# shubhamchandak94/Spring

Hardware: AMD Instinct MI355X
Metric: Mreads/s through reorder stage (higher is better)
Workload: dtype u64; 1 GPU; 100000000 x 150 bp single-end synthetic reads per GPU (uniform genome 600000000 bp, 25x coverage, 1.0% substitutions, 50% reverse-complemented), inputs resident in HBM as .dna records; reads_per_gpu=100000000, read_len=150, chains=65536, num_thr=8, parallelism=single GPU, unmatched=13958636, singletons=12720853, rounds=1984, chain_groups=2

## Files before the change

### include/spring_reorder.h

```cpp
#ifndef SPRING_REORDER_H_
#define SPRING_REORDER_H_

#include <stddef.h>
#include <stdint.h>

#ifdef __cplusplus
extern "C" {
#endif

#define SPRING_REORDER_E_ARG (-1)
#define SPRING_REORDER_E_IO (-2)
#define SPRING_REORDER_E_HIP (-3)
#define SPRING_REORDER_E_STATE (-4)

typedef struct spring_reorder_ctx spring_reorder_ctx;

typedef struct {
  int32_t device;
  uint32_t num_chains;
  int32_t num_thr;
  int32_t collect_stats;
  int32_t time_search;
  int32_t force_literal_update;
  int32_t rounds_per_sync;
// ... 22 lines not shown
  int32_t phases;
  int32_t known_absent;
  int32_t sort_prefix_bits;
  int32_t dict_build_mode;
  int32_t strand_filter;
} spring_reorder_opts;

typedef struct {
  uint64_t n_reads, n_matched, n_single, unmatched;
  uint64_t probes, keyok, cands, hits, iterations, rounds, lost;
  uint64_t numkeys[2], dict_numreads[2];
  double ms_unpack, ms_dict, ms_chains, ms_finalize, ms_total;
  double ms_search_kernel;
  uint64_t search_launches;
  uint64_t device_bytes;
  double ms_exchange, ms_resolve_mark;
  uint64_t chains;
  uint64_t deep_pool;
  uint64_t long_searches;
  uint64_t table_minz;
  uint64_t table_marked_lines;
  uint64_t long_splits;
  uint64_t alternatives;
  uint64_t phases;
  double ms_search_busy;
  uint64_t sort_prefix_bits;
  uint64_t sort_repaired_runs;
  uint64_t sort_full_sorts;
  uint64_t sort_long_runs;
  uint64_t sort_list_overflows;
  uint64_t dict_build_path;
  uint64_t strand_filter;
  uint64_t strand_filter_dropped;
} spring_reorder_stats;

void spring_reorder_default_opts(spring_reorder_opts *o);
const char *spring_reorder_last_error(void);
void spring_reorder_trim_pool(void);

int spring_reorder_run(const char *temp_dir, uint32_t max_readlen, int32_t num_thr, int32_t paired_end,
                       uint32_t num_reads_clean_0, uint32_t num_reads_clean_1,
                       const spring_reorder_opts *opts );

int spring_reorder_create(spring_reorder_ctx **ctx, const spring_reorder_opts *opts);
void spring_reorder_destroy(spring_reorder_ctx *ctx);

int spring_reorder_load_dna(spring_reorder_ctx *ctx, const uint8_t *dna, size_t nbytes, uint32_t n,
                            uint32_t max_readlen);

int spring_reorder_load_dna_device(spring_reorder_ctx *ctx, const void *d_dna, size_t nbytes, uint32_t n,
                                   uint32_t max_readlen, int32_t fixed_len);

int spring_reorder_build_dict(spring_reorder_ctx *ctx);

int spring_reorder_run_chains(spring_reorder_ctx *ctx);
int spring_reorder_auto_chains(spring_reorder_ctx *ctx, uint32_t *chains, int32_t *deep);

typedef struct {
  uint32_t num_reads[2], num_reads_clean[2], num_reads_N[2];
  uint32_t max_readlen;
  uint32_t pad;
  double ms_device;
} spring_fastq_info;
int spring_reorder_load_fastq(spring_reorder_ctx *ctx, const uint8_t *fastq_1, size_t nbytes_1, const uint8_t *fastq_2,
                              size_t nbytes_2 , spring_fastq_info *info);
int spring_reorder_fastq_N(spring_reorder_ctx *ctx, int32_t which, uint8_t *n_dna, size_t cap, size_t *nbytes,
// ... 4 lines not shown
int spring_reorder_mg_slice(spring_reorder_ctx *ctx, void **d_prop, size_t *slice_off, size_t *slice_bytes,
                            size_t *total_bytes);
int spring_reorder_mg_slices(spring_reorder_ctx *ctx, void **d_prop, size_t slice_off[2], size_t slice_bytes[2],
                             size_t *total_bytes, uint32_t *count);
int spring_reorder_mg_apply(spring_reorder_ctx *ctx, int32_t check_alive, uint32_t *alive);
int spring_reorder_mg_end(spring_reorder_ctx *ctx);
int spring_reorder_debug_check_seed_state(spring_reorder_ctx *ctx, int32_t group, uint64_t *violations);
int spring_reorder_mg_exchange_virtual(spring_reorder_ctx **ctxs, uint32_t world);

#define SPRING_RCCL_ID_BYTES 128
typedef struct spring_mg_comm spring_mg_comm;
typedef int (*spring_mg_allgather_fn)(void *host_buf, size_t slice_off, size_t slice_bytes, size_t total_bytes,
                                      void *user);
int spring_mg_rccl_unique_id(void *id128);
int spring_mg_comm_create_rccl(spring_mg_comm **comm, int32_t device, const void *id128, uint32_t rank, uint32_t world);
int spring_mg_comm_create_host(spring_mg_comm **comm, spring_mg_allgather_fn fn, void *user, uint32_t rank,
                               uint32_t world);
void spring_mg_comm_destroy(spring_mg_comm *comm);
int spring_reorder_mg_run(spring_reorder_ctx *ctx, spring_mg_comm *comm, uint32_t total_chains);

int spring_reorder_finalize(spring_reorder_ctx *ctx);

int spring_reorder_get_stats(spring_reorder_ctx *ctx, spring_reorder_stats *st);

int spring_reorder_download(spring_reorder_ctx *ctx, uint32_t *order, char *rc, char *flag, int64_t *pos,
                            uint16_t *rlen, uint32_t *order_s, uint64_t *tid_off, uint64_t *tid_off_s);
int spring_reorder_tid_split(spring_reorder_ctx *ctx, uint64_t *mid, uint64_t *mid_s);

int spring_reorder_emit_dna(spring_reorder_ctx *ctx, int32_t tid, uint8_t *dst, size_t cap, size_t *nbytes);

int spring_reorder_dict_lookup(spring_reorder_ctx *ctx, int32_t which, const uint64_t *keys, uint32_t nkeys,
                               uint32_t *bin_size, uint32_t *bin_ids, size_t ids_cap);

int spring_reorder_download_reads(spring_reorder_ctx *ctx, uint64_t *limbs , uint16_t *len);

int spring_order_invert_se(const uint32_t *order, uint32_t n, uint32_t *order_array, double *kernel_ms);
int spring_order_invert_pe(const uint32_t *order, uint32_t n, uint32_t *order_array, double *kernel_ms);
int spring_order_correct(uint32_t *order, uint64_t m, const uint32_t *order_N, uint32_t nN, uint32_t n_clean,
                         double *kernel_ms);
int spring_order_pe_encode(const uint32_t *order, uint32_t n, uint32_t *new_order, double *kernel_ms);

int spring_fastq_reorder(const uint8_t *fastq, size_t nbytes, const uint32_t *order, uint32_t n, uint8_t *out,
                         size_t out_cap, size_t *out_bytes, double *kernel_ms);

#define SPRING_SYNTH_REPEATS 0x80000000u
#define SPRING_SYNTH_PAIRED 0x40000000u
#define SPRING_SYNTH_GENOMIC 0x20000000u
size_t spring_synth_dna_bytes(uint32_t n, uint32_t L);
int spring_synth_dna_host(uint8_t *dst, uint32_t n, uint32_t L, uint64_t G, uint64_t seed, uint32_t err_ppm);
int spring_synth_genome_host(uint8_t *dst, uint64_t G, uint64_t seed, uint32_t flags);
int spring_synth_dna_device(void *d_dst, uint32_t n, uint32_t L, uint64_t G, uint64_t seed, uint32_t err_ppm);
int spring_reorder_load_synth(spring_reorder_ctx *ctx, uint32_t n, uint32_t L, uint64_t G, uint64_t seed,
                              uint32_t err_ppm);
int spring_reorder_download_dna(spring_reorder_ctx *ctx, uint8_t *dst, size_t cap);

#ifdef __cplusplus
}
#endif
#endif
```

### spring_amd/_lib.py

```python
import ctypes as C
import os

HERE = os.path.dirname(os.path.abspath(__file__))
LIB_PATH = os.environ.get("SPRING_AMD_LIB") or os.path.join(HERE, "lib", "libspring_reorder_hip.so")

EXPORTS = [
    "spring_reorder_default_opts", "spring_reorder_last_error", "spring_reorder_trim_pool", "spring_reorder_run", "spring_reorder_create",
    "spring_reorder_destroy", "spring_reorder_load_dna", "spring_reorder_load_dna_device",
    "spring_reorder_build_dict", "spring_reorder_run_chains", "spring_reorder_auto_chains", "spring_reorder_finalize",
    "spring_reorder_mg_begin", "spring_reorder_mg_search", "spring_reorder_mg_slice", "spring_reorder_mg_slices",
    "spring_reorder_mg_apply",
    "spring_reorder_mg_end", "spring_reorder_mg_exchange_virtual", "spring_reorder_debug_check_seed_state",
    "spring_mg_rccl_unique_id", "spring_mg_comm_create_rccl", "spring_mg_comm_create_host", "spring_mg_comm_destroy",
    "spring_reorder_mg_run",
    "spring_reorder_get_stats", "spring_reorder_download", "spring_reorder_tid_split", "spring_reorder_emit_dna",
    "spring_reorder_dict_lookup", "spring_reorder_download_reads", "spring_synth_dna_bytes",
    "spring_reorder_load_fastq", "spring_reorder_fastq_N",
    "spring_order_invert_se", "spring_order_invert_pe", "spring_order_correct", "spring_order_pe_encode",
    "spring_fastq_reorder",
    "spring_synth_dna_host", "spring_synth_genome_host", "spring_synth_dna_device", "spring_reorder_load_synth", "spring_reorder_download_dna",
    "spring_encoder_create", "spring_encoder_destroy", "spring_encoder_set_split_tables", "spring_encoder_encode_reorder", "spring_encoder_download",
    "spring_encoder_download_seq_packed", "spring_encoder_get_info", "spring_reorder_encode_run", "spring_encoder_encode_host", "spring_encoder_run",
]

STREAMS_EXPORTS = [
    "spring_streams_create", "spring_streams_destroy", "spring_streams_from_encoder", "spring_streams_from_host",
    "spring_streams_download", "spring_streams_get_info", "spring_streams_run",
]
STREAMS_NUM = 9

DECODE_EXPORTS = [
    "spring_decode_create", "spring_decode_destroy", "spring_decode_seq_from_encoder", "spring_decode_seq_from_host",
    "spring_decode_seq_from_files", "spring_decode_from_streams", "spring_decode_from_host", "spring_decode_from_files",
    "spring_decode_download", "spring_decode_get_info",
]

QUALID_EXPORTS = [
    "spring_qualid_create", "spring_qualid_destroy", "spring_qualid_order_from_host", "spring_qualid_order_from_encoder",
    "spring_qualid_from_fastq", "spring_qualid_from_lines", "spring_qualid_download", "spring_qualid_get_info",
    "spring_quality_table", "spring_id_pattern",
]

FASTQ_OUT_EXPORTS = [
    "spring_fastq_out_create", "spring_fastq_out_destroy", "spring_fastq_out_assemble", "spring_fastq_out_download",
    "spring_fastq_out_write", "spring_fastq_out_get_info",
]

GZIP_EXPORTS = [
    "spring_gzip_create", "spring_gzip_destroy", "spring_gzip_set_chunk_bytes", "spring_gzip_set_token_bytes",
# ... 132 lines not shown
        for k, _ in self._fields_:
            v = getattr(self, k)
            d[k] = list(v) if hasattr(v, "__len__") else v
        return d


class DecodeInfo(C.Structure):
    _fields_ = ([(k, C.c_uint64) for k in ("seq_len", "first_block", "num_blocks", "num_units")]
                + [("bases", C.c_uint64 * 2)]
                + [(k, C.c_uint64) for k in ("n_aligned", "n_unaligned", "pos_escapes")]
                + [("ms_device", C.c_double), ("ms_file", C.c_double)])

    def asdict(self):
        d = {}
        for k, _ in self._fields_:
            v = getattr(self, k)
            d[k] = list(v) if hasattr(v, "__len__") else v
        return d


class Stats(C.Structure):
    _fields_ = ([(k, C.c_uint64) for k in ("n_reads", "n_matched", "n_single", "unmatched", "probes", "keyok",
                                          "cands", "hits", "iterations", "rounds", "lost")]
                + [("numkeys", C.c_uint64 * 2), ("dict_numreads", C.c_uint64 * 2)]
                + [(k, C.c_double) for k in ("ms_unpack", "ms_dict", "ms_chains", "ms_finalize", "ms_total",
                                             "ms_search_kernel")]
                + [("search_launches", C.c_uint64), ("device_bytes", C.c_uint64),
                   ("ms_exchange", C.c_double), ("ms_resolve_mark", C.c_double), ("chains", C.c_uint64),
                   ("deep_pool", C.c_uint64), ("long_searches", C.c_uint64),
                   ("table_minz", C.c_uint64), ("table_marked_lines", C.c_uint64), ("long_splits", C.c_uint64), ("alternatives", C.c_uint64), ("phases", C.c_uint64),
                   ("ms_search_busy", C.c_double),
                   ("sort_prefix_bits", C.c_uint64), ("sort_repaired_runs", C.c_uint64), ("sort_full_sorts", C.c_uint64),
                   ("sort_long_runs", C.c_uint64), ("sort_list_overflows", C.c_uint64), ("dict_build_path", C.c_uint64),
                   ("strand_filter", C.c_uint64), ("strand_filter_dropped", C.c_uint64)])

    def asdict(self):
        d = {}
        for k, _ in self._fields_:
            v = getattr(self, k)
            d[k] = list(v) if hasattr(v, "__len__") else v
        return d


MG_ALLGATHER_FN = C.CFUNCTYPE(C.c_int, C.c_void_p, C.c_size_t, C.c_size_t, C.c_size_t, C.c_void_p)

_lib = None


def lib():
    global _lib
    if _lib is not None:
        return _lib
    if not os.path.exists(LIB_PATH):
        raise RuntimeError(
            "spring_amd: %s is missing. Build it with `python -m spring_amd.build` "
            "(or __graft_entry__.build()); there is no CPU fallback." % LIB_PATH)
    L = C.CDLL(LIB_PATH)
    vp, u8p = C.c_void_p, C.c_void_p
    L.spring_reorder_default_opts.argtypes = [C.POINTER(Opts)]
    L.spring_reorder_last_error.restype = C.c_char_p
    L.spring_reorder_trim_pool.restype = None
    L.spring_reorder_run.argtypes = [C.c_char_p, C.c_uint32, C.c_int32, C.c_int32, C.c_uint32, C.c_uint32,
                                     C.POINTER(Opts)]
    L.spring_reorder_create.argtypes = [C.POINTER(vp), C.POINTER(Opts)]
    L.spring_reorder_destroy.argtypes = [vp]
    L.spring_reorder_destroy.restype = None
    L.spring_reorder_load_dna.argtypes = [vp, u8p, C.c_size_t, C.c_uint32, C.c_uint32]
    L.spring_reorder_load_dna_device.argtypes = [vp, vp, C.c_size_t, C.c_uint32, C.c_uint32, C.c_int32]
    L.spring_reorder_build_dict.argtypes = [vp]
    L.spring_reorder_run_chains.argtypes = [vp]
    L.spring_reorder_auto_chains.argtypes = [vp, C.POINTER(C.c_uint32), C.POINTER(C.c_int32)]
    L.spring_reorder_finalize.argtypes = [vp]
    L.spring_reorder_mg_begin.argtypes = [vp, C.c_uint32, C.c_uint32, C.c_uint32, vp]
    L.spring_reorder_mg_search.argtypes = [vp]
    L.spring_reorder_mg_slice.argtypes = [vp, C.POINTER(vp), C.POINTER(C.c_size_t), C.POINTER(C.c_size_t), C.POINTER(C.c_size_t)]
    L.spring_reorder_mg_slices.argtypes = [vp, C.POINTER(vp), C.POINTER(C.c_size_t), C.POINTER(C.c_size_t), C.POINTER(C.c_size_t),
                                           C.POINTER(C.c_uint32)]
    L.spring_reorder_debug_check_seed_state.argtypes = [vp, C.c_int32, C.POINTER(C.c_uint64)]
    L.spring_reorder_mg_apply.argtypes = [vp, C.c_int32, C.POINTER(C.c_uint32)]
    L.spring_reorder_mg_end.argtypes = [vp]
    L.spring_reorder_mg_exchange_virtual.argtypes = [C.POINTER(vp), C.c_uint32]
    L.spring_mg_rccl_unique_id.argtypes = [vp]
    L.spring_mg_comm_create_rccl.argtypes = [C.POINTER(vp), C.c_int32, vp, C.c_uint32, C.c_uint32]
    L.spring_mg_comm_create_host.argtypes = [C.POINTER(vp), MG_ALLGATHER_FN, vp, C.c_uint32, C.c_uint32]
    L.spring_mg_comm_destroy.argtypes = [vp]
    L.spring_mg_comm_destroy.restype = None
    L.spring_reorder_mg_run.argtypes = [vp, vp, C.c_uint32]
    L.spring_reorder_get_stats.argtypes = [vp, C.POINTER(Stats)]
    L.spring_reorder_download.argtypes = [vp] + [vp] * 8
    L.spring_reorder_tid_split.argtypes = [vp, vp, vp]
    L.spring_reorder_emit_dna.argtypes = [vp, C.c_int32, u8p, C.c_size_t, C.POINTER(C.c_size_t)]
    L.spring_reorder_dict_lookup.argtypes = [vp, C.c_int32, vp, C.c_uint32, vp, vp, C.c_size_t]
    L.spring_reorder_download_reads.argtypes = [vp, vp, vp]
    L.spring_reorder_load_fastq.argtypes = [vp, vp, C.c_size_t, vp, C.c_size_t, C.POINTER(FastqInfo)]
    L.spring_reorder_fastq_N.argtypes = [vp, C.c_int32, vp, C.c_size_t, C.POINTER(C.c_size_t), vp, C.POINTER(C.c_uint32)]
    L.spring_order_invert_se.argtypes = [vp, C.c_uint32, vp, C.POINTER(C.c_double)]
    L.spring_order_invert_pe.argtypes = [vp, C.c_uint32, vp, C.POINTER(C.c_double)]
    L.spring_fastq_reorder.argtypes = [u8p, C.c_size_t, vp, C.c_uint32, u8p, C.c_size_t, C.POINTER(C.c_size_t),
                                       C.POINTER(C.c_double)]
    L.spring_order_pe_encode.argtypes = [vp, C.c_uint32, vp, C.POINTER(C.c_double)]
    L.spring_order_correct.argtypes = [vp, C.c_uint64, vp, C.c_uint32, C.c_uint32, C.POINTER(C.c_double)]
    L.spring_synth_dna_bytes.restype = C.c_size_t
    L.spring_synth_dna_bytes.argtypes = [C.c_uint32, C.c_uint32]
    L.spring_synth_dna_host.argtypes = [u8p, C.c_uint32, C.c_uint32, C.c_uint64, C.c_uint64, C.c_uint32]
    L.spring_synth_genome_host.argtypes = [u8p, C.c_uint64, C.c_uint64, C.c_uint32]
    L.spring_synth_dna_device.argtypes = [vp, C.c_uint32, C.c_uint32, C.c_uint64, C.c_uint64, C.c_uint32]
    L.spring_reorder_load_synth.argtypes = [vp, C.c_uint32, C.c_uint32, C.c_uint64, C.c_uint64, C.c_uint32]
    L.spring_reorder_download_dna.argtypes = [vp, u8p, C.c_size_t]
    L.spring_encoder_create.argtypes = [C.c_int32, C.POINTER(vp)]
    L.spring_encoder_destroy.argtypes = [vp]
    L.spring_encoder_destroy.restype = None
    L.spring_encoder_encode_reorder.argtypes = [vp, vp, u8p, C.c_uint64, vp, C.c_uint32, C.POINTER(EncoderInfo)]
    L.spring_encoder_download.argtypes = [vp] + [vp] * 9
    L.spring_encoder_download_seq_packed.argtypes = [vp, vp, vp]
    L.spring_encoder_encode_host.argtypes = [vp, C.c_uint32, C.c_int32, vp, u8p, C.c_uint64, vp, vp, vp, vp, vp, u8p,
                                             C.c_uint64, vp, C.c_uint32, u8p, C.c_uint64, vp, C.c_uint32,
                                             C.POINTER(EncoderInfo)]
    L.spring_encoder_run.argtypes = [C.c_char_p, C.c_uint32, C.c_int32, C.c_uint32, C.c_uint32, C.c_int32,
                                     C.POINTER(EncoderInfo)]
    L.spring_encoder_get_info.argtypes = [vp, C.POINTER(EncoderInfo)]
    L.spring_reorder_encode_run.argtypes = [C.c_char_p, C.c_uint32, C.c_int32, C.c_int32, C.c_uint32, C.c_uint32,
                                            C.c_uint32, C.POINTER(Opts), C.POINTER(EncoderInfo)]
    L.spring_streams_create.argtypes = [C.c_int32, C.POINTER(vp)]
    L.spring_streams_destroy.argtypes = [vp]
    L.spring_streams_destroy.restype = None
# ... 105 lines not shown
```

### spring_amd/csrc/dict_build.h

```cpp
#ifndef SPRING_DICT_BUILD_H_
#define SPRING_DICT_BUILD_H_

#include "reorder_device.h"

namespace sr {

bool launch_unpack_keys(hipStream_t st, const uint8_t *dna, uint32_t n, int L, int W, int S, uint32_t rec_fixed,
                        uint64_t *reads, uint16_t *lens, uint32_t *bad_len, int dstart0, int dend0, int dstart1, int dend1,
                        uint64_t *keys0, uint32_t *vals0, uint64_t *keys1, uint32_t *vals1);

constexpr int TAB_WRITE_LG = 10;
inline int tab_write_lg(int bshift) { return 64 - bshift < TAB_WRITE_LG ? 64 - bshift : TAB_WRITE_LG; }
inline uint32_t tab_write_blocks(int bshift) { return (uint32_t)(1ull << (64 - bshift - tab_write_lg(bshift))); }
void launch_tab_partition(hipStream_t st, const uint64_t *h0, uint32_t nk0, const uint64_t *h1, uint32_t nk1, int bshift,
                          uint32_t *part);
constexpr uint32_t TAB_OVF_SLOTS = 8;
void launch_tab_write(hipStream_t st, const uint64_t *h0, uint32_t nk0, const uint64_t *h1, uint32_t nk1,
                      const uint32_t *part, DictBuild d0, DictBuild d1, uint4 *fpt, int bshift, uint32_t *ovf,
                      uint32_t *ovf_blk, uint32_t *ovf_cnt);
void launch_tab_overflow_blocks(hipStream_t st, const uint64_t *h0, uint32_t nk0, const uint64_t *h1, DictBuild d0,
                                DictBuild d1, uint32_t *fpt, int bshift, const uint32_t *ovf_blk, const uint32_t *ovf_cnt);
void launch_tab_overflow_pairs(hipStream_t st, const uint64_t *h0, uint32_t nk0, const uint64_t *h1, DictBuild d0,
                               DictBuild d1, uint32_t *fpt, int bshift, const uint32_t *ovf, uint32_t novf);

constexpr uint32_t PRES_DROP_CTRS = 1024;
void launch_pres_insert(hipStream_t st, const uint64_t *h0, uint32_t nk0, const uint64_t *h1, uint32_t nk1, int wl, uint32_t *pres,
                        int lgb, uint32_t *drops);

}

#endif
```

### spring_amd/csrc/dict_build.hip

```cpp
#include <hip/hip_runtime.h>

#include "dict_build.h"
#include "strand_filter.h"

namespace sr {

__device__ __forceinline__ uint64_t db_mix64(uint64_t x) {
  x ^= x >> 33; x *= 0xff51afd7ed558ccdull; x ^= x >> 33; x *= 0xc4ceb9fe1a85ec53ull; x ^= x >> 33;
  return x;
}
__device__ __forceinline__ uint64_t db_unmix64(uint64_t x) {
  x ^= x >> 33; x *= 0x9cb4b2f8129337dbull; x ^= x >> 33; x *= 0x4f74430c22a54005ull; x ^= x >> 33;
  return x;
}
__device__ __forceinline__ uint32_t db_fp30_of(uint64_t h) {
  const uint32_t f = (uint32_t)h & 0x3fffffffu;
  return f == 0u ? 1u : f == 0x3fffffffu ? 0x3ffffffeu : f;
}

__global__ __launch_bounds__(256) void k_unpack_fixed_keys(const uint8_t *__restrict__ dna, uint32_t n, int L, int W, int lgS,
                                                           uint32_t rec, uint64_t *__restrict__ reads,
                                                           uint16_t *__restrict__ lens, uint32_t *__restrict__ bad_len,
                                                           int dstart0, int klen0, int dstart1, int klen1,
                                                           uint64_t *__restrict__ keys0, uint32_t *__restrict__ vals0,
// ... 56 lines not shown
  for (uint32_t r = threadIdx.x; r < nr; r += 256) {
    const uint32_t i = r0 + r;
    keys0[i] = db_mix64(window(r, dstart0, 2 * klen0));
    vals0[i] = i;
    keys1[i] = db_mix64(window(r, dstart1, 2 * klen1));
    vals1[i] = i;
  }
}

bool launch_unpack_keys(hipStream_t st, const uint8_t *dna, uint32_t n, int L, int W, int S, uint32_t rec_fixed,
                        uint64_t *reads, uint16_t *lens, uint32_t *bad_len, int dstart0, int dend0, int dstart1, int dend1,
                        uint64_t *keys0, uint32_t *vals0, uint64_t *keys1, uint32_t *vals1) {
  if (!n || ((uintptr_t)reads & 15u) || ((uintptr_t)lens & 3u)) return false;
  if (dstart0 < 0 || dstart1 < 0 || dend0 >= L || dend1 >= L || 2 * dend0 / 64 >= S || 2 * dend1 / 64 >= S) return false;
  int lgS = 0;
  while ((1 << lgS) < S) lgS++;
  const size_t lds = ((size_t)UNPACK_READS * rec_fixed + 15 + 12 + 15) / 16 * 16;
  hipLaunchKernelGGL(k_unpack_fixed_keys, dim3((n + UNPACK_READS - 1) / UNPACK_READS), dim3(256), lds, st, dna, n, L, W, lgS,
                     rec_fixed, reads, lens, bad_len, dstart0, dend0 - dstart0 + 1, dstart1, dend1 - dstart1 + 1, keys0, vals0,
                     keys1, vals1);
  return true;
}

__global__ void k_tab_partition(const uint64_t *__restrict__ h0, uint32_t nk0, const uint64_t *__restrict__ h1, uint32_t nk1,
                                int bshift, int lg, uint32_t nblk, uint32_t *__restrict__ part) {
  const uint64_t t = (uint64_t)blockIdx.x * blockDim.x + threadIdx.x;
  if (t >= 2ull * ((uint64_t)nblk + 1)) return;
  const uint32_t l = t > nblk ? 1u : 0u, j = (uint32_t)(t - (l ? (uint64_t)nblk + 1 : 0));
  const uint64_t *__restrict__ h = l ? h1 : h0;
  const uint32_t nk = l ? nk1 : nk0;
  uint32_t lo = 0, hi = nk;
  if (j == nblk) {
    lo = nk;
  } else {
    const uint64_t bound = ((uint64_t)j << lg) << bshift;
    while (lo < hi) {
      const uint32_t mid = lo + (hi - lo) / 2;
      if (h[mid] < bound) lo = mid + 1; else hi = mid;
    }
  }
  part[t] = lo;
}

constexpr uint32_t TAB_WRITE_TILE = 512, TAB_WRITE_THREADS = 512;
__global__ __launch_bounds__(TAB_WRITE_THREADS) void k_tab_write(const uint64_t *__restrict__ h0, uint32_t nk0,
                                                                 const uint64_t *__restrict__ h1, uint32_t nk1,
                                                                 const uint32_t *__restrict__ part, uint32_t nblk,
                                                                 DictBuild d0, DictBuild d1, uint4 *__restrict__ fpt,
                                                                 int bshift, int lg, uint32_t *__restrict__ ovf,
                                                                 uint32_t *__restrict__ ovf_blk, uint32_t *__restrict__ ovf_cnt) {
  __shared__ uint4 img[2u << TAB_WRITE_LG];
  __shared__ uint64_t tile[2][TAB_WRITE_TILE];
  __shared__ uint16_t first[2][1u << TAB_WRITE_LG];
  __shared__ uint32_t s_novf;
  const uint32_t nbk = 1u << lg, bmask = nbk - 1u, blk = blockIdx.x;
  for (uint32_t k = threadIdx.x; k < 2u * nbk; k += TAB_WRITE_THREADS) img[k] = make_uint4(0u, 0u, 0u, 0u);
  for (uint32_t k = threadIdx.x; k < nbk / 2u + 1u; k += TAB_WRITE_THREADS) {
    if (2u * k < nbk) { reinterpret_cast<uint32_t *>(first[0])[k] = 0u; reinterpret_cast<uint32_t *>(first[1])[k] = 0u; }
  }
  if (threadIdx.x == 0) s_novf = 0u;
  const uint32_t a0 = part[blk], a1 = part[(uint64_t)nblk + 1 + blk];
  const uint32_t c0 = part[blk + 1] - a0, c1 = part[(uint64_t)nblk + 2 + blk] - a1;
  const uint32_t ntot = c0 + c1;
  auto bin_of = [&](uint32_t t, uint32_t &st, uint32_t &cn, uint32_t &pay) {
    const bool l = t >= c0;
    const uint32_t i = l ? a1 + (t - c0) : a0 + t;
    st = (l ? d1.ustart : d0.ustart)[i]; cn = (l ? d1.ucount : d0.ucount)[i];
// ... 108 lines not shown
                                     DictBuild d0, DictBuild d1, uint32_t *fpt, int bshift, const uint32_t *__restrict__ ovf) {
  const uint32_t t = blockIdx.x * blockDim.x + threadIdx.x;
  if (t >= ovf[0]) return;
  tab_overflow_insert(ovf[1u + t], h0, nk0, h1, d0, d1, fpt, bshift);
}

void launch_tab_partition(hipStream_t st, const uint64_t *h0, uint32_t nk0, const uint64_t *h1, uint32_t nk1, int bshift,
                          uint32_t *part) {
  const uint32_t nblk = tab_write_blocks(bshift);
  const uint64_t nt = 2ull * ((uint64_t)nblk + 1);
  hipLaunchKernelGGL(k_tab_partition, dim3((unsigned)((nt + 255) / 256)), dim3(256), 0, st, h0, nk0, h1, nk1, bshift,
                     tab_write_lg(bshift), nblk, part);
}
void launch_tab_write(hipStream_t st, const uint64_t *h0, uint32_t nk0, const uint64_t *h1, uint32_t nk1,
                      const uint32_t *part, DictBuild d0, DictBuild d1, uint4 *fpt, int bshift, uint32_t *ovf,
                      uint32_t *ovf_blk, uint32_t *ovf_cnt) {
  const uint32_t nblk = tab_write_blocks(bshift);
  hipLaunchKernelGGL(k_tab_write, dim3(nblk), dim3(TAB_WRITE_THREADS), 0, st, h0, nk0, h1, nk1, part, nblk, d0, d1, fpt, bshift,
                     tab_write_lg(bshift), ovf, ovf_blk, ovf_cnt);
}
void launch_tab_overflow_blocks(hipStream_t st, const uint64_t *h0, uint32_t nk0, const uint64_t *h1, DictBuild d0,
                                DictBuild d1, uint32_t *fpt, int bshift, const uint32_t *ovf_blk, const uint32_t *ovf_cnt) {
  const uint32_t nblk = tab_write_blocks(bshift);
  const uint64_t nt = (uint64_t)nblk * TAB_OVF_SLOTS;
  hipLaunchKernelGGL(k_tab_overflow_blocks, dim3((unsigned)((nt + 255) / 256)), dim3(256), 0, st, h0, nk0, h1, d0, d1, fpt, bshift,
                     nblk, ovf_blk, ovf_cnt);
}
void launch_tab_overflow_pairs(hipStream_t st, const uint64_t *h0, uint32_t nk0, const uint64_t *h1, DictBuild d0,
                               DictBuild d1, uint32_t *fpt, int bshift, const uint32_t *ovf, uint32_t novf) {
  if (!novf) return;
  hipLaunchKernelGGL(k_tab_overflow_pairs, dim3((novf + 255) / 256), dim3(256), 0, st, h0, nk0, h1, d0, d1, fpt, bshift, ovf);
}

__global__ __launch_bounds__(256) void k_pres_insert(const uint64_t *__restrict__ h0, uint32_t nk0, const uint64_t *__restrict__ h1,
                                                     uint32_t nk1, int wl, uint32_t *__restrict__ pres, int lgb,
                                                     uint32_t *__restrict__ drops) {
  __shared__ uint32_t s_drop;
  if (threadIdx.x == 0) s_drop = 0u;
  __syncthreads();
  const uint64_t t = (uint64_t)blockIdx.x * blockDim.x + threadIdx.x;
  if (t < (uint64_t)nk0 + nk1) {
    const int l = t >= nk0 ? 1 : 0;
    const uint64_t key = db_unmix64(l ? h1[t - nk0] : h0[t]);
    uint32_t flags;
    const uint64_t hc = sf::mix64(sf::canon_and_flags(key, wl, l, flags));
    const uint32_t fp = sf::fp_of(hc), word = (fp << 4) | flags;
    uint32_t *bk = pres + 4ull * sf::bucket_of(hc, lgb);
    bool placed = false;
    for (int sl = 0; sl < 4 && !placed; sl++) {
      uint32_t old = __hip_atomic_load(bk + sl, __ATOMIC_RELAXED, __HIP_MEMORY_SCOPE_AGENT);
      if (old == 0u) old = atomicCAS(bk + sl, 0u, word);
      if (old == 0u) placed = true;
      else if ((old >> 4) == fp) {
        if ((old & word & 15u) != (word & 15u)) atomicOr(bk + sl, word & 15u);
        placed = true;
      }
    }
    if (!placed) atomicAdd(&s_drop, 1u);
  }
  __syncthreads();
  if (threadIdx.x == 0 && s_drop) atomicAdd(drops + (blockIdx.x & (PRES_DROP_CTRS - 1u)), s_drop);
}
void launch_pres_insert(hipStream_t st, const uint64_t *h0, uint32_t nk0, const uint64_t *h1, uint32_t nk1, int wl, uint32_t *pres,
                        int lgb, uint32_t *drops) {
  const uint64_t nt = (uint64_t)nk0 + nk1;
  if (!nt) return;
  hipLaunchKernelGGL(k_pres_insert, dim3((unsigned)((nt + 255) / 256)), dim3(256), 0, st, h0, nk0, h1, nk1, wl, pres, lgb, drops);
}

}
```

### spring_amd/csrc/reorder_pipeline.cpp

```cpp
#include <hip/hip_runtime.h>
#include <dlfcn.h>

#include <algorithm>
#include <system_error>
#include <thread>
#include <memory>
#include <atomic>
#include <chrono>
#include <cstdarg>
#include <cstdio>
#include <cstdlib>
#include <cstring>
#include <map>
#include <mutex>
#include <new>
#include <stdexcept>
#include <string>
#include <unordered_map>
#include <vector>
#include <zlib.h>

#include "reorder_device.h"
#include "dict_build.h"
#include "reorder_internal.h"
// ... 965 lines not shown
  HIPCHK(hipStreamSynchronize(ctx->st));
  if (!ctx->n) return 0;
  if (limbs)
    HIPCHK(hipMemcpy2D(limbs, (size_t)ctx->W * 8, ctx->d_reads, (size_t)ctx->S * 8, (size_t)ctx->W * 8, ctx->n,
                       hipMemcpyDeviceToHost));
  if (len) HIPCHK(hipMemcpy(len, ctx->d_lens, (size_t)ctx->n * 2, hipMemcpyDeviceToHost));
  return 0;
}

static uint64_t pow2ceil(uint64_t x) {
  uint64_t p = 1;
  while (p < x) p <<= 1;
  return p;
}

static double now_ms() {
  return std::chrono::duration<double, std::milli>(std::chrono::steady_clock::now().time_since_epoch()).count();
}
#define DBG_T(label)                                                                         \
  do {                                                                                       \
    if (dbg) { (void)hipStreamSynchronize(st); double t_ = now_ms(); fprintf(stderr, "[dict] %-14s %8.2f ms\n", label, t_ - t_last); t_last = t_; } \
  } while (0)

static TabView tab_view(const spring_reorder_ctx *ctx) {
  TabView t;
  t.buck = ctx->fpt;
  t.bshift = ctx->bshift; t.minz = ctx->minz; t.lshift = ctx->lshift;
  return t;
}

static unsigned sort_prefix_auto(uint64_t m) { return m <= (1ull << 29) ? 40u : 48u; }

static bool strand_filter_wanted(const spring_reorder_ctx *ctx);
int spring_reorder_build_dict(spring_reorder_ctx *ctx) {
  double t_last = now_ms();
  if (!ctx) return fail(SPRING_REORDER_E_ARG, "ctx is NULL");
  const bool dbg = ctx->o.debug != 0;
  if (ctx->stage != ST_LOADED) return fail(SPRING_REORDER_E_STATE, "build_dict: load reads first");
  HIPCHK(hipSetDevice(ctx->dev));
  hipStream_t st = ctx->st;
  const uint32_t n = ctx->n;
  HIPCHK(hipEventRecord(ctx->ev[2], st));
  uint64_t *uhash[2] = {nullptr, nullptr};
  uint32_t *ustart[2] = {nullptr, nullptr}, *ucount[2] = {nullptr, nullptr};
  const bool both_dense = n && ctx->uniform && ctx->L > ctx->dict[0].end && ctx->L > ctx->dict[1].end;
  uint64_t *keys_both[2] = {nullptr, nullptr};
  uint32_t *vals_both[2] = {nullptr, nullptr};
  ctx->stats.dict_build_path = 0;
  if (both_dense && ctx->pre_keys[0] && ctx->o.dict_build_mode != 1) {
    for (int l = 0; l < 2; l++) {
      keys_both[l] = ctx->pre_keys[l]; vals_both[l] = ctx->pre_vals[l];
      ctx->pre_keys[l] = nullptr; ctx->pre_vals[l] = nullptr;
    }
    ctx->stats.dict_build_path |= 1;
  } else {
    drop_pre_keys(ctx);
  }
  ctx->stats.sort_repaired_runs = 0; ctx->stats.sort_full_sorts = 0; ctx->stats.sort_prefix_bits = 0;
  ctx->stats.sort_long_runs = 0; ctx->stats.sort_list_overflows = 0;
  for (int l = 0; l < 2; l++) {
    DictDev &d = ctx->dict[l];
    uint32_t m = 0;
    uint32_t *d_slot = nullptr, *d_flag = nullptr;
    void *d_tmp = nullptr;
    size_t tmp_bytes = 0;
    if (n) {
      if (ctx->uniform) {
        m = ctx->L > d.end ? n : 0;
      } else {
        DMALLOC(d_flag, (size_t)n * 4);
        DMALLOC(d_slot, (size_t)n * 4);
        launch_flag_in_dict(st, ctx->d_lens, n, d.end, d_flag);
        HIPCHK(excl_scan_u32(st, nullptr, tmp_bytes, d_flag, d_slot, n));
        DMALLOC(d_tmp, tmp_bytes);
        HIPCHK(excl_scan_u32(st, d_tmp, tmp_bytes, d_flag, d_slot, n));
// ... 201 lines not shown
      DBG_T("insert pass 0");
      launch_tab_overflow(st, h_in, v_in, nm, db[0], db[1], tab_words, ctx->bshift, d_ovf, novf);
      if (dbg) fprintf(stderr, "[dict] %u of %llu pairs overflow their bucket\n", novf, (unsigned long long)nm);
    } else {
      DMALLOC(bk_in, nm * 4); DMALLOC(bk_out, nm * 4);
      DMALLOC(tp_in, nm * 8); DMALLOC(tp_out, nm * 8);
      launch_minz_prepare(st, h_in, v_in, nm, db[0], db[1], ctx->lshift, bk_in, tp_in);
      DBG_T("minz prepare");
      const unsigned end_bit = (unsigned)(64 - ctx->bshift);
      size_t tb = 0;
      HIPCHK(sort_pairs_u32_u64(st, nullptr, tb, bk_in, bk_out, tp_in, tp_out, nm, end_bit));
      DMALLOC(d_tmp2, tb);
      HIPCHK(sort_pairs_u32_u64(st, d_tmp2, tb, bk_in, bk_out, tp_in, tp_out, nm, end_bit));
      DBG_T("minz sort");
      DMALLOC(d_marked, 16);
      HIPCHK(hipMemsetAsync(d_marked, 0, 4, st));
      launch_tab_insert_minz(st, bk_out, tp_out, nm, tab_words, ctx->bshift, d_marked);
      HIPCHK(hipMemcpyAsync(&ctx->marked_lines, d_marked, 4, hipMemcpyDeviceToHost, st));
    }
    HIPCHK(hipGetLastError());
    uint32_t nd[2][3] = {{0, 0, 0}, {0, 0, 0}};
    for (int l = 0; l < 2; l++)
      HIPCHK(hipMemcpyAsync(nd[l], ctx->dict[l].d_ndeep, 12, hipMemcpyDeviceToHost, st));
    HIPCHK(hipStreamSynchronize(st));
    for (int l = 0; l < 2; l++) { ctx->dict[l].ndeep = nd[l][0]; ctx->dict[l].big_reads = nd[l][1]; ctx->dict[l].mid_reads = nd[l][2]; }
    if (dbg) fprintf(stderr, "[dict] reads %u + %u, keys %u + %u, bins >= %u: %u + %u, reads in bins >= %u: %u + %u, >= %u: %u + %u\n",
                     ctx->dict[0].numreads, ctx->dict[1].numreads, ctx->dict[0].numkeys, ctx->dict[1].numkeys, DEEP_BIN, nd[0][0], nd[1][0],
                     MID_BIN, nd[0][2], nd[1][2], BIG_BIN, nd[0][1], nd[1][1]);
    ctx->stats.table_marked_lines = ctx->marked_lines;
    DBG_T("insert");
    ctx->dfree(mv0); ctx->dfree(mh); ctx->dfree(mv); ctx->dfree(d_tmp);
    ctx->dfree(bk_in); ctx->dfree(bk_out); ctx->dfree(tp_in); ctx->dfree(tp_out); ctx->dfree(d_tmp2); ctx->dfree(d_marked); ctx->dfree(d_ovf);
  }
  ctx->pres = nullptr; ctx->pres_lgb = 0;
  ctx->stats.strand_filter = 0; ctx->stats.strand_filter_dropped = 0;
  int lgb = 0;
  if (nm && nm < 0xffffffffull && strand_filter_wanted(ctx)) {
    while (lgb < 32 && (1ull << lgb) < nm) lgb++;
    if (ctx->o.strand_filter > 0) lgb = std::min(lgb, ctx->o.strand_filter);
    if (ctx->dmalloc((void **)&ctx->pres, (size_t)16 << lgb)) {
      (void)hipGetLastError();
      ctx->pres = nullptr;
      if (dbg) fprintf(stderr, "[dict] presence table: no room for 2^%d buckets, running without\n", lgb);
    }
  }
  if (ctx->pres) {
    uint32_t *d_drops = nullptr;
    std::vector<uint32_t> h_drops(PRES_DROP_CTRS);
    DMALLOC(d_drops, PRES_DROP_CTRS * 4);
    HIPCHK(hipMemsetAsync(ctx->pres, 0, (size_t)16 << lgb, st));
    HIPCHK(hipMemsetAsync(d_drops, 0, PRES_DROP_CTRS * 4, st));
    launch_pres_insert(st, uhash[0], (uint32_t)nk0, uhash[1], (uint32_t)nk1, ctx->dict[0].end - ctx->dict[0].start + 1,
                       reinterpret_cast<uint32_t *>(ctx->pres), lgb, d_drops);
    HIPCHK(hipGetLastError());
    HIPCHK(hipMemcpyAsync(h_drops.data(), d_drops, PRES_DROP_CTRS * 4, hipMemcpyDeviceToHost, st));
    HIPCHK(hipStreamSynchronize(st));
    for (uint32_t v : h_drops) ctx->stats.strand_filter_dropped += v;
    ctx->pres_lgb = lgb;
    ctx->dfree(d_drops);
    if (dbg) fprintf(stderr, "[dict] presence table: 2^%d buckets, %llu of %llu keys dropped\n", lgb,
                     (unsigned long long)ctx->stats.strand_filter_dropped, (unsigned long long)nm);
    DBG_T("presence table");
  }
  for (int l = 0; l < 2; l++) { ctx->dfree(uhash[l]); ctx->dfree(ustart[l]); ctx->dfree(ucount[l]); }
  DBG_T("free temps");
  HIPCHK(hipEventRecord(ctx->ev[3], st));
  ctx->stage = ST_DICT;
  return 0;
}

int spring_reorder_dict_lookup(spring_reorder_ctx *ctx, int32_t which, const uint64_t *keys, uint32_t nkeys,
                               uint32_t *bin_size, uint32_t *bin_ids, size_t ids_cap) {
  if (!ctx || ctx->stage < ST_DICT) return fail(SPRING_REORDER_E_STATE, "dict_lookup: build_dict first");
  if (which < 0 || which > 1) return fail(SPRING_REORDER_E_ARG, "which must be 0 or 1");
  HIPCHK(hipSetDevice(ctx->dev));
  DictDev &d = ctx->dict[which];
  uint64_t *dk = nullptr;
  uint32_t *ds = nullptr, *dc = nullptr;
  DMALLOC(dk, (size_t)nkeys * 8);
  DMALLOC(ds, (size_t)nkeys * 4);
  DMALLOC(dc, (size_t)nkeys * 4);
  std::vector<uint32_t> hs(nkeys), hc(nkeys), hids(d.numreads);
  if (nkeys) {
    HIPCHK(hipMemcpyAsync(dk, keys, (size_t)nkeys * 8, hipMemcpyHostToDevice, ctx->st));
    launch_dict_lookup(ctx->st, tab_view(ctx), d.urec, which, ctx->d_reads, ctx->S, d.start, d.end, dk, nkeys, ds, dc);
    HIPCHK(hipMemcpyAsync(hs.data(), ds, (size_t)nkeys * 4, hipMemcpyDeviceToHost, ctx->st));
    HIPCHK(hipMemcpyAsync(hc.data(), dc, (size_t)nkeys * 4, hipMemcpyDeviceToHost, ctx->st));
  }
  if (d.numreads) HIPCHK(hipMemcpyAsync(hids.data(), d.ids, (size_t)d.numreads * 4, hipMemcpyDeviceToHost, ctx->st));
  HIPCHK(hipStreamSynchronize(ctx->st));
  ctx->dfree(dk); ctx->dfree(ds); ctx->dfree(dc);
  size_t o = 0;
  for (uint32_t i = 0; i < nkeys; i++) {
    if (hc[i] != 0xffffffffu && (hc[i] & 0x80000000u)) {
      bin_size[i] = 1;
      if (o + 1 > ids_cap) return fail(SPRING_REORDER_E_ARG, "bin_ids too small");
      bin_ids[o++] = hs[i];
      continue;
    }
    bin_size[i] = hc[i];
    if (hc[i] == 0xffffffffu) continue;
    if (o + hc[i] > ids_cap) return fail(SPRING_REORDER_E_ARG, "bin_ids too small");
    memcpy(bin_ids + o, hids.data() + hs[i], (size_t)hc[i] * 4);
    o += hc[i];
  }
  return 0;
}

static bool dict_is_deep(const spring_reorder_ctx *ctx) {
  const uint64_t nd = (uint64_t)ctx->dict[0].numreads + ctx->dict[1].numreads, nk = (uint64_t)ctx->dict[0].numkeys + ctx->dict[1].numkeys;
  return nd * 10 >= nk * 13;
}
static bool dict_has_heavy_tail(const spring_reorder_ctx *ctx) {
  const uint64_t mid = (uint64_t)ctx->dict[0].mid_reads + ctx->dict[1].mid_reads, nd = (uint64_t)ctx->dict[0].numreads + ctx->dict[1].numreads;
  return nd > 0 && mid * 1000 >= nd;
}
static bool dict_is_contended(const spring_reorder_ctx *ctx) {
  const uint64_t mid = (uint64_t)ctx->dict[0].mid_reads + ctx->dict[1].mid_reads, nd = (uint64_t)ctx->dict[0].numreads + ctx->dict[1].numreads;
  return nd > 0 && mid * 4 >= nd;
}
static bool dict_wants_deep_kernel(const spring_reorder_ctx *ctx) {
  const uint64_t nd = (uint64_t)ctx->dict[0].numreads + ctx->dict[1].numreads, nk = (uint64_t)ctx->dict[0].numkeys + ctx->dict[1].numkeys;
  return nd * 100 >= nk * 115 || dict_has_heavy_tail(ctx);
}
static bool dict_is_very_deep(const spring_reorder_ctx *ctx) {
  const uint64_t big = (uint64_t)ctx->dict[0].big_reads + ctx->dict[1].big_reads, nd = (uint64_t)ctx->dict[0].numreads + ctx->dict[1].numreads;
  return dict_is_deep(ctx) && nd > 0 && big * 4 >= nd;
}
static bool ka_layout_ok(const spring_reorder_ctx *ctx, int *ka_lo) {
  if (ctx->Lpad > 192 || ctx->o.known_absent < 0 || ctx->minz) return false;
  const int wlen = ctx->dict[0].end - ctx->dict[0].start + 1, lo = ctx->dict[0].start >> 5;
  if (wlen <= 32 && ctx->dict[1].start == ctx->dict[0].end + 1 && ctx->dict[1].end - ctx->dict[1].start + 1 == wlen &&
      2 * (ctx->L - wlen) + 2 <= 64 * (lo + 4) && 2 * ctx->dict[1].start + 2 <= 256 && lo + 4 <= 6) {
    if (ka_lo) *ka_lo = lo;
    return true;
  }
  return false;
}
// ... 1314 lines not shown
```

### spring_amd/reorder.py

```python
import ctypes as C
from dataclasses import dataclass

import numpy as np

from . import _lib


class ReorderError(RuntimeError):
    """Raised where the reference throws std::runtime_error (call_template_functions.cpp:60)."""


@dataclass
class ReorderOpts:
    device: int = -1
    num_chains: int = 0
    num_thr: int = 1
    collect_stats: bool = False
    time_search: bool = False
    force_literal_update: bool = False
    rounds_per_sync: int = 0
    first_shifts: int = 0
    seed_wide: int = 0
    tab_scale: int = 0
    search_wpb: int = 0
# ... 150 lines not shown

    def streams(self):
        st = self.stats()
        nm, ns, T = st["n_matched"], st["n_single"], self.opts.num_thr
        out = dict(order=np.zeros(max(nm, 1), np.uint32), rc=np.zeros(max(nm, 1), np.uint8),
                   flag=np.zeros(max(nm, 1), np.uint8), pos=np.zeros(max(nm, 1), np.int64),
                   rlen=np.zeros(max(nm, 1), np.uint16), order_s=np.zeros(max(ns, 1), np.uint32),
                   tid_off=np.zeros(T + 1, np.uint64), tid_off_s=np.zeros(T + 1, np.uint64))
        _chk(self._L.spring_reorder_download(self._h, *[out[k].ctypes.data for k in (
            "order", "rc", "flag", "pos", "rlen", "order_s", "tid_off", "tid_off_s")]))
        for k in ("order", "rc", "flag", "pos", "rlen"):
            out[k] = out[k][:nm]
        out["order_s"] = out["order_s"][:ns]
        out["tid_mid"], out["tid_mid_s"] = np.zeros(T, np.uint64), np.zeros(T, np.uint64)
        _chk(self._L.spring_reorder_tid_split(self._h, out["tid_mid"].ctypes.data, out["tid_mid_s"].ctypes.data))
        out["stats"] = st
        return out

    def emit_dna(self, tid: int) -> bytes:
        nb = C.c_size_t()
        _chk(self._L.spring_reorder_emit_dna(self._h, tid, None, 0, C.byref(nb)))
        buf = np.zeros(max(nb.value, 1), np.uint8)
        _chk(self._L.spring_reorder_emit_dna(self._h, tid, buf.ctypes.data, nb.value, C.byref(nb)))
        return buf[:nb.value].tobytes()

    def dict_lookup(self, which, keys):
        keys = np.ascontiguousarray(keys, dtype=np.uint64)
        sizes = np.zeros(max(len(keys), 1), np.uint32)
        ids = np.zeros(max(self.n, 1) * 2, np.uint32)
        _chk(self._L.spring_reorder_dict_lookup(self._h, which, keys.ctypes.data, len(keys), sizes.ctypes.data,
                                                ids.ctypes.data, len(ids)))
        return sizes[:len(keys)], ids

    def download_reads(self):
        W = (2 * self.max_readlen - 1) // 64 + 1
        limbs = np.zeros((max(self.n, 1), W), np.uint64)
        ln = np.zeros(max(self.n, 1), np.uint16)
        _chk(self._L.spring_reorder_download_reads(self._h, limbs.ctypes.data, ln.ctypes.data))
        return limbs[:self.n], ln[:self.n]

    def download_dna(self) -> bytes:
        nb = self._L.spring_synth_dna_bytes(self.n, self.max_readlen)
        buf = np.zeros(max(nb, 1), np.uint8)
        _chk(self._L.spring_reorder_download_dna(self._h, buf.ctypes.data, nb))
        p = 0
        for _ in range(self.n):
            p += 2 + ((int(buf[p]) | (int(buf[p + 1]) << 8)) + 3) // 4
        return buf[:p].tobytes()


def reorder_dna(dna: bytes, n: int, max_readlen: int, opts: ReorderOpts = None):
    with ReorderStage(opts) as s:
        s.load_dna(dna, n, max_readlen)
        return s.run().streams()


def synth_dna_host(n, L, G, seed, err_ppm=10000) -> bytes:
    L_ = _lib.lib()
    nb = L_.spring_synth_dna_bytes(n, L)
    buf = np.zeros(max(nb, 1), np.uint8)
    _chk(L_.spring_synth_dna_host(buf.ctypes.data, n, L, G, seed, err_ppm))
    return buf[:nb].tobytes()


SYNTH_REPEATS = 0x80000000
SYNTH_PAIRED = 0x40000000
# ... 27 lines not shown
```

Baseline: 366.6 Mreads/s.

## Build presence table per block in LDS and write each bucket range once

When the dictionary is built in one pass, the strand-filter presence table is no longer zeroed with a memset and filled by global atomics. Keys are first partitioned by bucket range, then each block assembles its slice of the table in shared memory and writes it out once; a second global-atomic pass handles only the cross-strand keys. This aims to cut the memset traffic and global atomic contention during table construction, at the cost of an extra partition kernel, a second pass over the keys, and a new download API for inspecting the table.

```diff
diff --git a/include/spring_reorder.h b/include/spring_reorder.h
--- a/include/spring_reorder.h
+++ b/include/spring_reorder.h
@@ -78,6 +78,7 @@
   uint64_t dict_build_path;
   uint64_t strand_filter;
   uint64_t strand_filter_dropped;
+  uint64_t strand_filter_build;
 } spring_reorder_stats;
 
 void spring_reorder_default_opts(spring_reorder_opts *o);
@@ -148,6 +149,8 @@
 int spring_reorder_dict_lookup(spring_reorder_ctx *ctx, int32_t which, const uint64_t *keys, uint32_t nkeys,
                                uint32_t *bin_size, uint32_t *bin_ids, size_t ids_cap);
 
+int spring_reorder_presence_table(spring_reorder_ctx *ctx, void *out, size_t cap, int32_t *lgb);
+
 int spring_reorder_download_reads(spring_reorder_ctx *ctx, uint64_t *limbs , uint16_t *len);
 
 int spring_order_invert_se(const uint32_t *order, uint32_t n, uint32_t *order_array, double *kernel_ms);
diff --git a/spring_amd/_lib.py b/spring_amd/_lib.py
--- a/spring_amd/_lib.py
+++ b/spring_amd/_lib.py
@@ -14,7 +14,7 @@
     "spring_mg_rccl_unique_id", "spring_mg_comm_create_rccl", "spring_mg_comm_create_host", "spring_mg_comm_destroy",
     "spring_reorder_mg_run",
     "spring_reorder_get_stats", "spring_reorder_download", "spring_reorder_tid_split", "spring_reorder_emit_dna",
-    "spring_reorder_dict_lookup", "spring_reorder_download_reads", "spring_synth_dna_bytes",
+    "spring_reorder_dict_lookup", "spring_reorder_presence_table", "spring_reorder_download_reads", "spring_synth_dna_bytes",
     "spring_reorder_load_fastq", "spring_reorder_fastq_N",
     "spring_order_invert_se", "spring_order_invert_pe", "spring_order_correct", "spring_order_pe_encode",
     "spring_fastq_reorder",
@@ -213,7 +213,8 @@
                    ("ms_search_busy", C.c_double),
                    ("sort_prefix_bits", C.c_uint64), ("sort_repaired_runs", C.c_uint64), ("sort_full_sorts", C.c_uint64),
                    ("sort_long_runs", C.c_uint64), ("sort_list_overflows", C.c_uint64), ("dict_build_path", C.c_uint64),
-                   ("strand_filter", C.c_uint64), ("strand_filter_dropped", C.c_uint64)])
+                   ("strand_filter", C.c_uint64), ("strand_filter_dropped", C.c_uint64),
+                   ("strand_filter_build", C.c_uint64)])
 
     def asdict(self):
         d = {}
@@ -272,6 +273,7 @@
     L.spring_reorder_tid_split.argtypes = [vp, vp, vp]
     L.spring_reorder_emit_dna.argtypes = [vp, C.c_int32, u8p, C.c_size_t, C.POINTER(C.c_size_t)]
     L.spring_reorder_dict_lookup.argtypes = [vp, C.c_int32, vp, C.c_uint32, vp, vp, C.c_size_t]
+    L.spring_reorder_presence_table.argtypes = [vp, vp, C.c_size_t, C.POINTER(C.c_int32)]
     L.spring_reorder_download_reads.argtypes = [vp, vp, vp]
     L.spring_reorder_load_fastq.argtypes = [vp, vp, C.c_size_t, vp, C.c_size_t, C.POINTER(FastqInfo)]
     L.spring_reorder_fastq_N.argtypes = [vp, C.c_int32, vp, C.c_size_t, C.POINTER(C.c_size_t), vp, C.POINTER(C.c_uint32)]
diff --git a/spring_amd/csrc/dict_build.h b/spring_amd/csrc/dict_build.h
--- a/spring_amd/csrc/dict_build.h
+++ b/spring_amd/csrc/dict_build.h
@@ -24,8 +24,13 @@
                                DictBuild d1, uint32_t *fpt, int bshift, const uint32_t *ovf, uint32_t novf);
 
 constexpr uint32_t PRES_DROP_CTRS = 1024;
+constexpr int PRES_WRITE_LG = 10;
+inline int pres_write_lg(int lgb) { return lgb < PRES_WRITE_LG ? lgb : PRES_WRITE_LG; }
+inline uint32_t pres_write_blocks(int lgb) { return 1u << (lgb - pres_write_lg(lgb)); }
 void launch_pres_insert(hipStream_t st, const uint64_t *h0, uint32_t nk0, const uint64_t *h1, uint32_t nk1, int wl, uint32_t *pres,
-                        int lgb, uint32_t *drops);
+                        int lgb, uint32_t *drops, bool skip_self_canonical);
+void launch_pres_write(hipStream_t st, const uint64_t *h0, uint32_t nk0, const uint64_t *h1, uint32_t nk1, int wl, uint4 *pres,
+                       int lgb, uint32_t *part, uint32_t *drops);
 
 }
 
diff --git a/spring_amd/csrc/dict_build.hip b/spring_amd/csrc/dict_build.hip
--- a/spring_amd/csrc/dict_build.hip
+++ b/spring_amd/csrc/dict_build.hip
@@ -112,7 +112,7 @@
   uint32_t lo = 0, hi = nk;
   if (j == nblk) {
     lo = nk;
-  } else {
+  } else if (j != 0u) {
     const uint64_t bound = ((uint64_t)j << lg) << bshift;
     while (lo < hi) {
       const uint32_t mid = lo + (hi - lo) / 2;
@@ -287,21 +287,64 @@
   hipLaunchKernelGGL(k_tab_overflow_pairs, dim3((novf + 255) / 256), dim3(256), 0, st, h0, nk0, h1, d0, d1, fpt, bshift, ovf);
 }
 
+constexpr uint32_t PRES_WRITE_THREADS = 256;
+__global__ __launch_bounds__(PRES_WRITE_THREADS) void k_pres_write(const uint64_t *__restrict__ h0, const uint64_t *__restrict__ h1,
+                                                                   const uint32_t *__restrict__ part, uint32_t nblk, int wl,
+                                                                   uint4 *__restrict__ pres, int lgb, int lg,
+                                                                   uint32_t *__restrict__ drops) {
+  __shared__ uint4 img[1u << PRES_WRITE_LG];
+  __shared__ uint32_t s_drop;
+  const uint32_t nbk = 1u << lg, bmask = nbk - 1u, blk = blockIdx.x;
+  for (uint32_t k = threadIdx.x; k < nbk; k += PRES_WRITE_THREADS) img[k] = make_uint4(0u, 0u, 0u, 0u);
+  if (threadIdx.x == 0) s_drop = 0u;
+  const uint32_t a0 = part[blk], a1 = part[(uint64_t)nblk + 1 + blk];
+  const uint32_t c0 = part[blk + 1] - a0, c1 = part[(uint64_t)nblk + 2 + blk] - a1;
+  const uint32_t ntot = c0 + c1;
+  __syncthreads();
+  uint32_t *imgw = reinterpret_cast<uint32_t *>(img);
+  for (uint32_t t = threadIdx.x; t < ntot; t += PRES_WRITE_THREADS) {
+    const int l = t >= c0 ? 1 : 0;
+    const uint64_t h = l ? h1[a1 + (t - c0)] : h0[a0 + t];
+    uint32_t flags;
+    const uint64_t cw = sf::canon_and_flags(db_unmix64(h), wl, l, flags);
+    if (!(flags & (1u << l))) continue;
+    const uint64_t hc = sf::mix64(cw);
+    const uint32_t fp = sf::fp_of(hc), word = (fp << 4) | flags;
+    uint32_t *bk = imgw + 4u * (sf::bucket_of(hc, lgb) & bmask);
+    bool placed = false;
+    for (int sl = 0; sl < 4 && !placed; sl++) {
+      const uint32_t old = atomicCAS(bk + sl, 0u, word);
+      if (old == 0u) placed = true;
+      else if ((old >> 4) == fp) {
+        if ((old & word & 15u) != (word & 15u)) atomicOr(bk + sl, word & 15u);
+        placed = true;
+      }
+    }
+    if (!placed) atomicAdd(&s_drop, 1u);
+  }
+  __syncthreads();
+  if (threadIdx.x == 0 && s_drop) atomicAdd(drops + (blk & (PRES_DROP_CTRS - 1u)), s_drop);
+  uint4 *__restrict__ out = pres + ((uint64_t)blk << lg);
+  for (uint32_t k = threadIdx.x; k < nbk; k += PRES_WRITE_THREADS) out[k] = img[k];
+}
 __global__ __launch_bounds__(256) void k_pres_insert(const uint64_t *__restrict__ h0, uint32_t nk0, const uint64_t *__restrict__ h1,
                                                      uint32_t nk1, int wl, uint32_t *__restrict__ pres, int lgb,
-                                                     uint32_t *__restrict__ drops) {
+                                                     uint32_t *__restrict__ drops, int skip_self) {
   __shared__ uint32_t s_drop;
   if (threadIdx.x == 0) s_drop = 0u;
   __syncthreads();
   const uint64_t t = (uint64_t)blockIdx.x * blockDim.x + threadIdx.x;
-  if (t < (uint64_t)nk0 + nk1) {
+  bool mine = t < (uint64_t)nk0 + nk1;
+  if (mine) {
     const int l = t >= nk0 ? 1 : 0;
     const uint64_t key = db_unmix64(l ? h1[t - nk0] : h0[t]);
     uint32_t flags;
-    const uint64_t hc = sf::mix64(sf::canon_and_flags(key, wl, l, flags));
+    const uint64_t cw = sf::canon_and_flags(key, wl, l, flags);
+    if (skip_self && (flags & (1u << l))) mine = false;
+    const uint64_t hc = sf::mix64(cw);
     const uint32_t fp = sf::fp_of(hc), word = (fp << 4) | flags;
     uint32_t *bk = pres + 4ull * sf::bucket_of(hc, lgb);
-    bool placed = false;
+    bool placed = !mine;
     for (int sl = 0; sl < 4 && !placed; sl++) {
       uint32_t old = __hip_atomic_load(bk + sl, __ATOMIC_RELAXED, __HIP_MEMORY_SCOPE_AGENT);
       if (old == 0u) old = atomicCAS(bk + sl, 0u, word);
@@ -317,10 +360,19 @@
   if (threadIdx.x == 0 && s_drop) atomicAdd(drops + (blockIdx.x & (PRES_DROP_CTRS - 1u)), s_drop);
 }
 void launch_pres_insert(hipStream_t st, const uint64_t *h0, uint32_t nk0, const uint64_t *h1, uint32_t nk1, int wl, uint32_t *pres,
-                        int lgb, uint32_t *drops) {
+                        int lgb, uint32_t *drops, bool skip_self_canonical) {
   const uint64_t nt = (uint64_t)nk0 + nk1;
   if (!nt) return;
-  hipLaunchKernelGGL(k_pres_insert, dim3((unsigned)((nt + 255) / 256)), dim3(256), 0, st, h0, nk0, h1, nk1, wl, pres, lgb, drops);
-}
-
-}
+  hipLaunchKernelGGL(k_pres_insert, dim3((unsigned)((nt + 255) / 256)), dim3(256), 0, st, h0, nk0, h1, nk1, wl, pres, lgb, drops,
+                     skip_self_canonical ? 1 : 0);
+}
+void launch_pres_write(hipStream_t st, const uint64_t *h0, uint32_t nk0, const uint64_t *h1, uint32_t nk1, int wl, uint4 *pres,
+                       int lgb, uint32_t *part, uint32_t *drops) {
+  const int lg = pres_write_lg(lgb);
+  const uint32_t nblk = pres_write_blocks(lgb);
+  const uint64_t nt = 2ull * ((uint64_t)nblk + 1);
+  hipLaunchKernelGGL(k_tab_partition, dim3((unsigned)((nt + 255) / 256)), dim3(256), 0, st, h0, nk0, h1, nk1, 64 - lgb, lg, nblk, part);
+  hipLaunchKernelGGL(k_pres_write, dim3(nblk), dim3(PRES_WRITE_THREADS), 0, st, h0, h1, part, nblk, wl, pres, lgb, lg, drops);
+}
+
+}
diff --git a/spring_amd/csrc/reorder_pipeline.cpp b/spring_amd/csrc/reorder_pipeline.cpp
--- a/spring_amd/csrc/reorder_pipeline.cpp
+++ b/spring_amd/csrc/reorder_pipeline.cpp
@@ -1021,6 +1021,19 @@
 static unsigned sort_prefix_auto(uint64_t m) { return m <= (1ull << 29) ? 40u : 48u; }
 
 static bool strand_filter_wanted(const spring_reorder_ctx *ctx);
+
+static bool presence_wanted(const spring_reorder_ctx *ctx, uint64_t nm) { return nm && nm < 0xffffffffull && strand_filter_wanted(ctx); }
+static int presence_alloc(spring_reorder_ctx *ctx, uint64_t nm, bool dbg) {
+  int lgb = 0;
+  while (lgb < 32 && (1ull << lgb) < nm) lgb++;
+  if (ctx->o.strand_filter > 0) lgb = std::min(lgb, ctx->o.strand_filter);
+  if (ctx->dmalloc((void **)&ctx->pres, (size_t)16 << lgb)) {
+    (void)hipGetLastError();
+    ctx->pres = nullptr;
+    if (dbg) fprintf(stderr, "[dict] presence table: no room for 2^%d buckets, running without\n", lgb);
+  }
+  return lgb;
+}
 int spring_reorder_build_dict(spring_reorder_ctx *ctx) {
   double t_last = now_ms();
   if (!ctx) return fail(SPRING_REORDER_E_ARG, "ctx is NULL");
@@ -1030,6 +1043,8 @@
   hipStream_t st = ctx->st;
   const uint32_t n = ctx->n;
   HIPCHK(hipEventRecord(ctx->ev[2], st));
+  ctx->pres = nullptr; ctx->pres_lgb = 0;
+  ctx->stats.strand_filter = 0; ctx->stats.strand_filter_dropped = 0; ctx->stats.strand_filter_build = 0;
   uint64_t *uhash[2] = {nullptr, nullptr};
   uint32_t *ustart[2] = {nullptr, nullptr}, *ucount[2] = {nullptr, nullptr};
   const bool both_dense = n && ctx->uniform && ctx->L > ctx->dict[0].end && ctx->L > ctx->dict[1].end;
@@ -1297,33 +1312,30 @@
     ctx->dfree(mv0); ctx->dfree(mh); ctx->dfree(mv); ctx->dfree(d_tmp);
     ctx->dfree(bk_in); ctx->dfree(bk_out); ctx->dfree(tp_in); ctx->dfree(tp_out); ctx->dfree(d_tmp2); ctx->dfree(d_marked); ctx->dfree(d_ovf);
   }
-  ctx->pres = nullptr; ctx->pres_lgb = 0;
-  ctx->stats.strand_filter = 0; ctx->stats.strand_filter_dropped = 0;
   int lgb = 0;
-  if (nm && nm < 0xffffffffull && strand_filter_wanted(ctx)) {
-    while (lgb < 32 && (1ull << lgb) < nm) lgb++;
-    if (ctx->o.strand_filter > 0) lgb = std::min(lgb, ctx->o.strand_filter);
-    if (ctx->dmalloc((void **)&ctx->pres, (size_t)16 << lgb)) {
-      (void)hipGetLastError();
-      ctx->pres = nullptr;
-      if (dbg) fprintf(stderr, "[dict] presence table: no room for 2^%d buckets, running without\n", lgb);
-    }
-  }
+  if (presence_wanted(ctx, nm)) lgb = presence_alloc(ctx, nm, dbg);
   if (ctx->pres) {
-    uint32_t *d_drops = nullptr;
+    const int wl = ctx->dict[0].end - ctx->dict[0].start + 1;
+    uint32_t *d_drops = nullptr, *d_part = nullptr;
     std::vector<uint32_t> h_drops(PRES_DROP_CTRS);
     DMALLOC(d_drops, PRES_DROP_CTRS * 4);
-    HIPCHK(hipMemsetAsync(ctx->pres, 0, (size_t)16 << lgb, st));
     HIPCHK(hipMemsetAsync(d_drops, 0, PRES_DROP_CTRS * 4, st));
-    launch_pres_insert(st, uhash[0], (uint32_t)nk0, uhash[1], (uint32_t)nk1, ctx->dict[0].end - ctx->dict[0].start + 1,
-                       reinterpret_cast<uint32_t *>(ctx->pres), lgb, d_drops);
+    if (one_pass) {
+      DMALLOC(d_part, 2 * ((size_t)pres_write_blocks(lgb) + 1) * 4);
+      launch_pres_write(st, uhash[0], (uint32_t)nk0, uhash[1], (uint32_t)nk1, wl, ctx->pres, lgb, d_part, d_drops);
+    } else {
+      HIPCHK(hipMemsetAsync(ctx->pres, 0, (size_t)16 << lgb, st));
+    }
+    launch_pres_insert(st, uhash[0], (uint32_t)nk0, uhash[1], (uint32_t)nk1, wl, reinterpret_cast<uint32_t *>(ctx->pres), lgb, d_drops,
+                       one_pass);
     HIPCHK(hipGetLastError());
     HIPCHK(hipMemcpyAsync(h_drops.data(), d_drops, PRES_DROP_CTRS * 4, hipMemcpyDeviceToHost, st));
     HIPCHK(hipStreamSynchronize(st));
     for (uint32_t v : h_drops) ctx->stats.strand_filter_dropped += v;
     ctx->pres_lgb = lgb;
-    ctx->dfree(d_drops);
-    if (dbg) fprintf(stderr, "[dict] presence table: 2^%d buckets, %llu of %llu keys dropped\n", lgb,
+    ctx->stats.strand_filter_build = one_pass ? 2 : 1;
+    ctx->dfree(d_drops); ctx->dfree(d_part);
+    if (dbg) fprintf(stderr, "[dict] presence table: 2^%d buckets%s, %llu of %llu keys dropped\n", lgb, one_pass ? " written once" : "",
                      (unsigned long long)ctx->stats.strand_filter_dropped, (unsigned long long)nm);
     DBG_T("presence table");
   }
@@ -1369,6 +1381,19 @@
     memcpy(bin_ids + o, hids.data() + hs[i], (size_t)hc[i] * 4);
     o += hc[i];
   }
+  return 0;
+}
+
+int spring_reorder_presence_table(spring_reorder_ctx *ctx, void *out, size_t cap, int32_t *lgb) {
+  if (!ctx || ctx->stage < ST_DICT) return fail(SPRING_REORDER_E_STATE, "presence_table: build_dict first");
+  if (!ctx->pres) return fail(SPRING_REORDER_E_STATE, "presence_table: this build made no presence table");
+  const size_t nb = (size_t)16 << ctx->pres_lgb;
+  if (lgb) *lgb = ctx->pres_lgb;
+  if (!out) return 0;
+  if (cap < nb) return fail(SPRING_REORDER_E_ARG, "presence_table: the table has %zu bytes, the buffer %zu", nb, cap);
+  HIPCHK(hipSetDevice(ctx->dev));
+  HIPCHK(hipMemcpyAsync(out, ctx->pres, nb, hipMemcpyDeviceToHost, ctx->st));
+  HIPCHK(hipStreamSynchronize(ctx->st));
   return 0;
 }
 
diff --git a/spring_amd/reorder.py b/spring_amd/reorder.py
--- a/spring_amd/reorder.py
+++ b/spring_amd/reorder.py
@@ -206,6 +206,13 @@
                                                 ids.ctypes.data, len(ids)))
         return sizes[:len(keys)], ids
 
+    def presence_table(self):
+        lgb = C.c_int32(0)
+        _chk(self._L.spring_reorder_presence_table(self._h, None, 0, C.byref(lgb)))
+        slots = np.zeros((1 << lgb.value, 4), np.uint32)
+        _chk(self._L.spring_reorder_presence_table(self._h, slots.ctypes.data, slots.nbytes, C.byref(lgb)))
+        return lgb.value, slots
+
     def download_reads(self):
         W = (2 * self.max_readlen - 1) // 64 + 1
         limbs = np.zeros((max(self.n, 1), W), np.uint64)
```

Result: faster. 370.4 Mreads/s, median of 6 (+1.0%).
